# lrjconan/LanczosNetwork

Measured on NVIDIA H100. Metric: QM8 molecules/sec (forward), higher is better.
Workload: dtype f32

## Files before the change

### lanczosnetwork_b200/csrc/sm90.cuh

```cuda
#pragma once
#include <cuda.h>
#include <cuda_runtime.h>
#include <stdint.h>

namespace sm90 {

__device__ __forceinline__ uint32_t smem_u32(const void* p) {
  return static_cast<uint32_t>(__cvta_generic_to_shared(p));
}

__device__ __forceinline__ void mbar_init(uint64_t* bar, uint32_t count) {
  asm volatile("mbarrier.init.shared::cta.b64 [%0], %1;" ::"r"(smem_u32(bar)), "r"(count));
}
__device__ __forceinline__ void fence_barrier_init() {
  asm volatile("fence.mbarrier_init.release.cluster;" ::: "memory");
}
__device__ __forceinline__ void mbar_arrive(uint64_t* bar) {
  asm volatile("mbarrier.arrive.shared::cta.b64 _, [%0];" ::"r"(smem_u32(bar)) : "memory");
}
__device__ __forceinline__ void mbar_arrive_expect_tx(uint64_t* bar, uint32_t bytes) {
  asm volatile("mbarrier.arrive.expect_tx.shared::cta.b64 _, [%0], %1;" ::"r"(smem_u32(bar)),
               "r"(bytes)
               : "memory");
}
// ... 81 lines not shown
        "setp.ne.and.b32 p, %1, 0, e;\n\t"
        "@p mbarrier.arrive.expect_tx.shared::cta.b64 _, [%0], %2;\n\t"
        "@p cp.async.bulk.tensor.2d.shared::cluster.global.mbarrier::complete_tx::bytes"
        " [%3], [%4, {%7, %8}], [%0];\n\t"
        "@p cp.async.bulk.tensor.2d.shared::cluster.global.mbarrier::complete_tx::bytes"
        " [%5], [%6, {%7, %8}], [%0];\n\t}"
        ::"r"(smem_u32(bar)), "r"((uint32_t)pred), "r"(bytes), "r"(smem_u32(dst0)),
          "l"(reinterpret_cast<uint64_t>(m0)), "r"(smem_u32(dst1)), "l"(reinterpret_cast<uint64_t>(m1)),
          "r"(c0), "r"(c1)
        : "memory");
  }
}

__device__ __forceinline__ bool elect_one() {
  uint32_t pred;
  asm volatile(
      "{\n\t.reg .pred p;\n\t"
      "elect.sync _|p, 0xffffffff;\n\t"
      "selp.b32 %0, 1, 0, p;\n\t}"
      : "=r"(pred));
  return pred != 0;
}

__device__ __forceinline__ uint32_t tf32_rna_bits(float v) {
  uint32_t r;
  asm("cvt.rna.tf32.f32 %0, %1;" : "=r"(r) : "f"(v));
  return r;
}

__device__ __forceinline__ uint64_t wgmma_desc_kmajor_sw128(uint32_t smem_addr) {
  uint64_t d = 0;
  d |= (uint64_t)((smem_addr >> 4) & 0x3FFFu);
  d |= (uint64_t)1 << 16;
  d |= (uint64_t)64 << 32;
  d |= (uint64_t)1 << 62;
  return d;
}
__device__ __forceinline__ void wgmma_fence() { asm volatile("wgmma.fence.sync.aligned;" ::: "memory"); }
__device__ __forceinline__ void wgmma_commit() { asm volatile("wgmma.commit_group.sync.aligned;" ::: "memory"); }
__device__ __forceinline__ void wgmma_wait_all() { asm volatile("wgmma.wait_group.sync.aligned 0;" ::: "memory"); }
__device__ __forceinline__ void wgmma_fence_operand(float (&d)[128]) {
#pragma unroll
  for (int i = 0; i < 128; ++i) asm volatile("" : "+f"(d[i])::"memory");
}
__device__ __forceinline__ void wgmma_wait_one() { asm volatile("wgmma.wait_group.sync.aligned 1;" ::: "memory"); }

// ... 47 lines not shown
```

### lanczosnetwork_b200/csrc/spectral_conv_fused.cu

```cuda
#include "tc_gemm.cuh"

namespace {

constexpr int KMAX = 32;
constexpr int GMAX = 32;
constexpr int RMAX = 128;
constexpr int EMAX = 16;
constexpr int FR = 8;

template <bool STAGE>
__global__ void __launch_bounds__(256)
graph_prepare_kernel(const float* __restrict__ L, const float* __restrict__ Q, int N, int E1, int K,
                     float* __restrict__ ell_val, uint8_t* __restrict__ ell_idx,
                     int32_t* __restrict__ ell_max, int32_t* __restrict__ gext, int binarize) {
  extern __shared__ __align__(16) float gp_smem[];
  __shared__ int s_max[EMAX];
  __shared__ int s_ext[2];
  __shared__ uint8_t cnt_s[256 * EMAX];
  const int b = blockIdx.x, tid = threadIdx.x;
  if (tid < EMAX) s_max[tid] = 0;
  if (tid < 2) s_ext[tid] = 0;
  const int64_t per = (int64_t)N * N * E1;
  const float* Lg = L + b * per;
  if (STAGE) {
// ... 375 lines not shown
    if (t < T2) { S[1 + t] = run + ex; tst[t] = run + ex; }
    run += tot;
  }
  if (tid == 0) { S[0] = T2; S[1 + T2] = B; }
  __syncthreads();
  for (int r = warp; r < nrec; r += 32) {
    const int sm = rec_sm[r];
    if (lane < (sm >> 8)) S[T2 + 2 + tst[rec_t[r]] + (sm & 255) + lane] = order[rec_src[r] + lane];
  }
}

constexpr int STACK_PLAIN = 0;
constexpr int STACK_SAGE_MEAN = 1;
constexpr int STACK_SAGE_MAX = 2;
constexpr float SAGE_EPS = 1.1920928955078125e-07f;

template <int kVariant>
struct SpectralPolicyT {
  static constexpr bool kNormRows = kVariant != STACK_PLAIN;
  static constexpr bool kMaxAgg = kVariant == STACK_SAGE_MAX;
  static constexpr bool kLongScales = kVariant == STACK_PLAIN;
  static constexpr int kStagesB = 2;
  static constexpr int kStagesA = 2;
  static constexpr int LMAX = 8;
  struct Params {
    const float* X;
    const int64_t* node_ids;
    const float* emb;
    const float* Q;
    const float* coeff;
    int64_t coeff_stride;
    const float* ell_val;
    const uint8_t* ell_idx;
    const int32_t* ell_max;
    const int32_t* gext;
    const int32_t* tiles;
    const float* bias;
    float* out;
    const float* W_out;
    const float* b_out;
    const float* w_att;
    const float* b_att;
    const uint8_t* mask;
    float* score;
    int P, emb_rows;
    int L;
// ... 31 lines not shown

  struct Tables {
    int ng, Rtot, Ztot, nquads, nzquads, nlines;
    int gid[GMAX];
    int nbase[GMAX + 1], kbase[GMAX + 1], gn[GMAX], gk[GMAX];
    int cnt_e[EMAX], base_e[EMAX], tmax_e[EMAX];
    uint8_t emax[GMAX][EMAX];
    uint8_t row_g[RMAX], row_n[RMAX], z_g[RMAX], z_k[RMAX];
    uint8_t q_g[RMAX / 4 + GMAX], q_n0[RMAX / 4 + GMAX];
    uint8_t zq_g[RMAX / 4 + GMAX], zq_k0[RMAX / 4 + GMAX];
    uint8_t line_e[256], line_t[256];
  };

  const Params& p;
  const int tid, r;
  const int N, K, S, E1, H, XP;
  int Din;
  Tables* tb;
  float* Xs;
  float* Qs;
  float* Ev;
  uint8_t* Ei;
  float fr[FR];
  float u[tcg::BK];
  float* ring;
  tcg::PhaseTimer* ptm = nullptr;

  static __host__ __device__ constexpr size_t tables_bytes() { return (sizeof(Tables) + 15) & ~size_t(15); }

  __device__ SpectralPolicyT(const Params& p_, uint8_t* smem, int tid_)
      : p(p_), tid(tid_), r(tid_ & 127), N(p_.N), K(p_.K), S(p_.S), E1(p_.E1),
        H(p_.H), XP(x_pitch(p_.Din[0], p_.H)), Din(p_.Din[0]) {
    tb = reinterpret_cast<Tables*>(smem);
    Xs = reinterpret_cast<float*>(smem + tables_bytes());
    Qs = Xs + (size_t)RMAX * XP;
    Ev = Qs + (size_t)RMAX * K;
    Ei = reinterpret_cast<uint8_t*>(Ev + (size_t)p.LB * RMAX);
    ring = reinterpret_cast<float*>(tcg::a_ring(smem, kStagesB, kStagesA));
  }
  static size_t smem_fixed(int Din, int K, int H) {
    return (size_t)RMAX * x_pitch(Din, H) * 4 + (size_t)RMAX * K * 4 + tables_bytes() + 16;
  }
  static size_t ell_line_bytes() { return (size_t)RMAX * 5; }
  static size_t readout_bytes(int H, int P, int N) {
    const size_t P1 = (size_t)P + 1, PQ = (P1 + 3) / 4, yr = (RMAX + 1) * P1;
    return (4 * PQ * (H + 4) + yr + ((4 - (yr & 3)) & 3) + H) * 4 + (size_t)GMAX * N;
  }

  __device__ void build_tables(int m_tile) {
    const int lane = tid & 31;
    const int32_t* sc = schedule(p);
// ... 34 lines not shown
        int m = em[e];
        if (lane < ng) tb->emax[lane][e] = (uint8_t)m;
#pragma unroll
        for (int o = 16; o > 0; o >>= 1) m = max(m, __shfl_xor_sync(0xffffffffu, m, o));
        if (lane == 0) tb->tmax_e[e] = m;
      }
    }
    __syncwarp();
    if (lane == 0) {
      tb->ng = ng; tb->Rtot = Rtot; tb->Ztot = Ztot; tb->nquads = nquads; tb->nzquads = nzquads;
      tb->nbase[ng] = Rtot; tb->kbase[ng] = Ztot;
      int left = p.LB, base = 0;
      for (int e = 0; e < E1; ++e) {
        const int c = min(tb->tmax_e[e], left);
        tb->cnt_e[e] = c; tb->base_e[e] = base;
        for (int t = 0; t < c; ++t) { tb->line_e[base + t] = (uint8_t)e; tb->line_t[base + t] = (uint8_t)t; }
        base += c; left -= c;
      }
      tb->nlines = base;
    }
  }

  __device__ void step_begin(int m_tile, int sub, int , tcg::PhaseTimer& tm) {
    tcg::producers_sync();
    const int layer = sub >> 1, step = sub & 1;
    if (step == 1 && S > 0) return;
    Din = p.Din[layer];
    const int warp = tid >> 5, lane = tid & 31;
    constexpr int NW = tcg::PRODUCER_THREADS / 32;
    const int dv = Din / 4;
    ptm = &tm;
    if (layer == 0) {
    if (warp == 0) build_tables(m_tile);
    tcg::producers_sync();
    tm.lap(16);
    const int Rtot = tb->Rtot;
    int64_t my_id = 0;
    if (!p.X && warp + lane * NW < Rtot) {
      const int row = warp + lane * NW;
      my_id = __ldg(p.node_ids + (int64_t)tb->gid[tb->row_g[row]] * N + tb->row_n[row]);
    }
    for (int row = warp, j = 0; row < Rtot; row += NW, ++j) {
      const int64_t src_row = (int64_t)tb->gid[tb->row_g[row]] * N + tb->row_n[row];
      const float* xsrc;
      if (p.X) {
        xsrc = p.X + src_row * Din;
      } else {
        int64_t id = __shfl_sync(0xffffffffu, my_id, j);
        id = id < 0 ? 0 : (id >= p.emb_rows ? p.emb_rows - 1 : id);
        xsrc = p.emb + id * Din;
      }
      float* xd = Xs + (size_t)row * XP;
      for (int q4 = lane; q4 < dv; q4 += 32) sm90::cp_async_16(xd + 4 * q4, xsrc + 4 * q4);
      const float* qsrc = p.Q + src_row * K;
      float* qd = Qs + (size_t)row * K;
      for (int k4 = lane; k4 < (K >> 2); k4 += 32) sm90::cp_async_16(qd + 4 * k4, qsrc + 4 * k4);
    }
// ... 24 lines not shown
          for (int u = 0; u < ELL_BATCH; ++u) {
            const int line = base + u * NW;
            if (line < nlines && rr < Rtot) {
              Ev[(size_t)line * RMAX + rr] = vv[u];
              Ei[(size_t)line * RMAX + rr] = (uint8_t)ii[u];
            }
          }
        }
      }
    }
    tm.lap(18);
    }
    const int Ztot = tb->Ztot;
#pragma unroll
    for (int i = 0; i < FR; ++i) fr[i] = 0.f;
    if (S > 0 && r < Ztot) {
      const float* f = p.coeff + layer * p.coeff_stride + ((int64_t)tb->gid[tb->z_g[r]] * K + tb->z_k[r]) * S;
#pragma unroll
      for (int i = 0; i < FR; ++i)
        if (i < S) fr[i] = __ldg(f + i);
    }
    tm.lap(0);
    sm90::cp_async_wait_all();
    tcg::producers_sync();
    tm.lap(1);
  }

  __device__ __forceinline__ void produce(int sub, int kb, float (&v)[32]) {
#pragma unroll
    for (int j = 0; j < 32; ++j) v[j] = 0.f;
    if (kLongScales && (sub & 1) == 0) {
      if (r >= tb->Ztot) return;
      const int s = kb % S;
      if (s == 0) {
        const int g = tb->z_g[r], n_g = tb->gn[g], nb = tb->nbase[g];
        const float* xs = Xs + (size_t)nb * XP + (kb / S) * tcg::BK;
        const float* qs = Qs + (size_t)nb * K + tb->z_k[r];
#pragma unroll
        for (int j = 0; j < tcg::BK; ++j) u[j] = 0.f;
#pragma unroll 2
        for (int n = 0; n < n_g; ++n) {
          const float q = qs[(size_t)n * K];
          const float4* x4 = reinterpret_cast<const float4*>(xs + (size_t)n * XP);
#pragma unroll
          for (int j = 0; j < 8; ++j) {
            const float4 t = x4[j];
            u[4 * j + 0] = fmaf(q, t.x, u[4 * j + 0]); u[4 * j + 1] = fmaf(q, t.y, u[4 * j + 1]);
            u[4 * j + 2] = fmaf(q, t.z, u[4 * j + 2]); u[4 * j + 3] = fmaf(q, t.w, u[4 * j + 3]);
          }
        }
      }
      float f = 0.f;
      if (S <= FR) {
#pragma unroll
        for (int i = 0; i < FR; ++i) f = (i == s) ? fr[i] : f;
      } else {
        f = __ldg(p.coeff + (sub >> 1) * p.coeff_stride + ((int64_t)tb->gid[tb->z_g[r]] * K + tb->z_k[r]) * S + s);
      }
#pragma unroll
      for (int j = 0; j < tcg::BK; ++j) v[j] = f * u[j];
      return;
    }
    const int j0 = kb * tcg::BK;
    const int c = j0 / Din, d0 = j0 - c * Din;
    if (r >= tb->Rtot) return;
    const int e = c;
    if constexpr (kMaxAgg) {
      produce_max(e, d0, v);
      return;
    }
    const float* xs = Xs + d0;
    const int ts = tb->cnt_e[e], tmax = tb->tmax_e[e];
    const float* ev = Ev + (size_t)tb->base_e[e] * RMAX + r;
    const uint8_t* ei = Ei + (size_t)tb->base_e[e] * RMAX + r;
#pragma unroll 2
    for (int t = 0; t < ts; ++t) {
      const float a = ev[t * RMAX];
      if (a == 0.f) continue;
      const int i = ei[t * RMAX];
      const float4* x4 = reinterpret_cast<const float4*>(xs + (size_t)i * XP);
#pragma unroll
      for (int q = 0; q < 8; ++q) {
        const float4 tt = x4[q];
        v[4 * q + 0] = fmaf(a, tt.x, v[4 * q + 0]);
        v[4 * q + 1] = fmaf(a, tt.y, v[4 * q + 1]);
        v[4 * q + 2] = fmaf(a, tt.z, v[4 * q + 2]);
        v[4 * q + 3] = fmaf(a, tt.w, v[4 * q + 3]);
      }
    }
    if (ts < tmax) {
      const int g = tb->row_g[r], n = tb->row_n[r];
      const int my = tb->emax[g][e], nb = tb->nbase[g];
      const int64_t off0 = (((int64_t)tb->gid[g] * E1 + e) * N) * N + n;
      for (int t = ts; t < tmax; ++t) {
        float a = 0.f;
        int i = 0;
        if (t < my) {
          a = __ldg(p.ell_val + off0 + (int64_t)t * N);
          i = nb + __ldg(p.ell_idx + off0 + (int64_t)t * N);
        }
        if (a == 0.f) continue;
        const float4* x4 = reinterpret_cast<const float4*>(xs + (size_t)i * XP);
#pragma unroll
        for (int q = 0; q < 8; ++q) {
          const float4 tt = x4[q];
          v[4 * q + 0] = fmaf(a, tt.x, v[4 * q + 0]);
          v[4 * q + 1] = fmaf(a, tt.y, v[4 * q + 1]);
          v[4 * q + 2] = fmaf(a, tt.z, v[4 * q + 2]);
          v[4 * q + 3] = fmaf(a, tt.w, v[4 * q + 3]);
        }
      }
    }
  }

  __device__ __forceinline__ void produce_max(int e, int d0, float (&v)[32]) {
#pragma unroll
    for (int j = 0; j < 32; ++j) v[j] = -INFINITY;
    bool any = false;
    const float* xs = Xs + d0;
    const int ts = tb->cnt_e[e], tmax = tb->tmax_e[e];
    const float* ev = Ev + (size_t)tb->base_e[e] * RMAX + r;
    const uint8_t* ei = Ei + (size_t)tb->base_e[e] * RMAX + r;
    for (int t = 0; t < ts; ++t) {
      if (ev[t * RMAX] == 0.f) continue;
      const float4* x4 = reinterpret_cast<const float4*>(xs + (size_t)ei[t * RMAX] * XP);
      any = true;
#pragma unroll
      for (int q = 0; q < 8; ++q) {
        const float4 tt = x4[q];
        v[4 * q + 0] = fmaxf(v[4 * q + 0], tt.x);
        v[4 * q + 1] = fmaxf(v[4 * q + 1], tt.y);
        v[4 * q + 2] = fmaxf(v[4 * q + 2], tt.z);
        v[4 * q + 3] = fmaxf(v[4 * q + 3], tt.w);
      }
    }
    if (ts < tmax) {
      const int g = tb->row_g[r], n = tb->row_n[r];
      const int my = tb->emax[g][e], nb = tb->nbase[g];
      const int64_t off0 = (((int64_t)tb->gid[g] * E1 + e) * N) * N + n;
      for (int t = ts; t < tmax && t < my; ++t) {
        if (__ldg(p.ell_val + off0 + (int64_t)t * N) == 0.f) continue;
        const int i = nb + __ldg(p.ell_idx + off0 + (int64_t)t * N);
        const float4* x4 = reinterpret_cast<const float4*>(xs + (size_t)i * XP);
        any = true;
#pragma unroll
        for (int q = 0; q < 8; ++q) {
          const float4 tt = x4[q];
          v[4 * q + 0] = fmaxf(v[4 * q + 0], tt.x);
          v[4 * q + 1] = fmaxf(v[4 * q + 1], tt.y);
          v[4 * q + 2] = fmaxf(v[4 * q + 2], tt.z);
          v[4 * q + 3] = fmaxf(v[4 * q + 3], tt.w);
        }
      }
    }
    if (!any) {
#pragma unroll
      for (int j = 0; j < 32; ++j) v[j] = 0.f;
    }
  }

  __device__ __forceinline__ void normalize_row(float* row) const {
    float4* r4 = reinterpret_cast<float4*>(row);
    float ss = 0.f;
    for (int h4 = 0; h4 < H / 4; ++h4) {
      const float4 t = r4[h4];
      ss = fmaf(t.x, t.x, ss); ss = fmaf(t.y, t.y, ss); ss = fmaf(t.z, t.z, ss); ss = fmaf(t.w, t.w, ss);
    }
    const float den = sqrtf(ss) + SAGE_EPS;
    for (int h4 = 0; h4 < H / 4; ++h4) {
      const float4 t = r4[h4];
      r4[h4] = make_float4(t.x / den, t.y / den, t.z / den, t.w / den);
    }
  }
  __device__ __forceinline__ float pad_den(const float* bias) const {
    float ss = 0.f;
    for (int h = 0; h < H; ++h) {
      float t = bias ? __ldg(bias + h) : 0.f;
      t = (p.relu != 0) ? fmaxf(t, 0.f) : t;
      ss = fmaf(t, t, ss);
    }
    return sqrtf(ss) + SAGE_EPS;
  }

  __device__ void pre_epilogue(int sub) {
    if ((sub & 1) == 0) return;
    tcg::producers_sync();
    if (ptm) ptm->lap(22);
  }

  static __device__ __forceinline__ bool acc_init(const Params& p, const uint8_t* smem, const float* zr,
                                                  int sub, int row0, int cl, float (&d)[128]) {
    if (!kLongScales || (sub & 1) == 0 || p.S == 0) return false;
    const Tables* tb = reinterpret_cast<const Tables*>(smem);
    const int K = p.K;
    const float* Qs = reinterpret_cast<const float*>(smem + tables_bytes()) + (size_t)RMAX * x_pitch(p.Din[0], p.H);
    const int Rtot = tb->Rtot;
#pragma unroll
    for (int i = 0; i < 128; ++i) d[i] = 0.f;
#pragma unroll
    for (int h = 0; h < 2; ++h) {
      const int row = row0 + 8 * h;
      if (row >= Rtot) continue;
      const int g = tb->row_g[row], k_g = tb->gk[g], zb = tb->kbase[g];
      const float* q = Qs + (size_t)row * K;
      for (int k = 0; k < k_g; ++k) {
        const float a = q[k];
#pragma unroll
        for (int j = 0; j < 16; ++j) {
          const float2 t = *reinterpret_cast<const float2*>(zr + tcg::stg_index(zb + k, 8 * j + cl, tcg::BN));
// ... 8 lines not shown
  __device__ __forceinline__ void store(int sub, int col, float (&x)[tcg::EW]) {
    if (col >= H || r >= tb->Rtot) return;
    float4* o4 = reinterpret_cast<float4*>(Xs + (size_t)r * XP + col);
    const bool relu = p.relu != 0;
    const float* bias = p.bias ? p.bias + (sub >> 1) * H : nullptr;
#pragma unroll
    for (int q = 0; q < tcg::EW / 4; ++q) {
      if (col + 4 * q >= H) break;
      float y[4] = {x[4 * q + 0], x[4 * q + 1], x[4 * q + 2], x[4 * q + 3]};
      if (bias) {
        const float4 b4 = __ldg(reinterpret_cast<const float4*>(bias + col) + q);
        y[0] += b4.x; y[1] += b4.y; y[2] += b4.z; y[3] += b4.w;
      }
      if (relu) { y[0] = fmaxf(y[0], 0.f); y[1] = fmaxf(y[1], 0.f); y[2] = fmaxf(y[2], 0.f); y[3] = fmaxf(y[3], 0.f); }
      o4[q] = make_float4(y[0], y[1], y[2], y[3]);
    }
  }

  __device__ void post_epilogue(int sub) {
    if constexpr (kNormRows) {
      if ((sub & 1) != 0 && r < tb->Rtot) normalize_row(Xs + (size_t)r * XP);
    }
    if ((sub & 1) == 0 || (sub >> 1) != p.L - 1) return;
    tcg::producers_sync();
    if (ptm) ptm->lap(19);
    const int warp = tid >> 5, lane = tid & 31;
    constexpr int NW = tcg::PRODUCER_THREADS / 32;
    const int hv = H / 4, Rtot = tb->Rtot;
    const float* bias = p.bias ? p.bias + (p.L - 1) * H : nullptr;
    if (p.out) {
      for (int row = warp; row < Rtot; row += NW) {
        const float4* src = reinterpret_cast<const float4*>(Xs + (size_t)row * XP);
        float4* dst = reinterpret_cast<float4*>(
            p.out + ((int64_t)tb->gid[tb->row_g[row]] * N + tb->row_n[row]) * H);
        for (int q4 = lane; q4 < hv; q4 += 32) dst[q4] = src[q4];
      }
      if (p.write_pad) {
        [[maybe_unused]] float den = 1.f;
        if constexpr (kNormRows) den = pad_den(bias);
        const int npad = tb->ng * N - Rtot;
        for (int i = warp; i < npad; i += NW) {
          int g = 0, rem = i;
          while (rem >= N - tb->gn[g]) { rem -= N - tb->gn[g]; ++g; }
          float4* dst = reinterpret_cast<float4*>(p.out + ((int64_t)tb->gid[g] * N + tb->gn[g] + rem) * H);
          for (int q4 = lane; q4 < hv; q4 += 32) {
            float y[4];
#pragma unroll
            for (int u = 0; u < 4; ++u) {
              float t = bias ? __ldg(bias + 4 * q4 + u) : 0.f;
              y[u] = (p.relu != 0) ? fmaxf(t, 0.f) : t;
              if constexpr (kNormRows) y[u] = y[u] / den;
            }
            dst[q4] = make_float4(y[0], y[1], y[2], y[3]);
          }
        }
      }
    }
    if (p.score) readout(bias);
  }

  __device__ void readout(const float* bias_last) {
    const int P = p.P, P1 = p.P + 1, PQ = (P1 + 3) >> 2, HP = H + 4;
    float* Wr = ring;
    float* Yr = Wr + (size_t)4 * PQ * HP;
    float* cx = Yr + (size_t)(RMAX + 1) * P1 + ((4 - ((RMAX + 1) * P1 & 3)) & 3);
    for (int e = tid; e < 4 * PQ * H; e += tcg::PRODUCER_THREADS) {
      const int o = e / H, h = e - o * H;
      Wr[o * HP + h] = (o < P) ? __ldg(p.W_out + o * H + h) : (o == P ? __ldg(p.w_att + h) : 0.f);
    }
    [[maybe_unused]] float den = 1.f;
    if constexpr (kNormRows) den = pad_den(bias_last);
    for (int h = tid; h < H; h += tcg::PRODUCER_THREADS) {
      float t = bias_last ? __ldg(bias_last + h) : 0.f;
      cx[h] = (p.relu != 0) ? fmaxf(t, 0.f) : t;
      if constexpr (kNormRows) cx[h] = cx[h] / den;
    }
    uint8_t* mk = reinterpret_cast<uint8_t*>(cx + H);
    for (int e = tid; e < tb->ng * N; e += tcg::PRODUCER_THREADS) {
      const int g = e / N;
      mk[e] = p.mask ? __ldg(p.mask + (int64_t)tb->gid[g] * N + (e - g * N)) : (uint8_t)1;
    }
    tcg::producers_sync();
    if (ptm) ptm->lap(20);
    const int Rtot = tb->Rtot;
    {
      const int warp = tid >> 5, lane = tid & 31;
      const int rb = warp & 3, og = warp >> 2;
      const int per = (P1 + tcg::NGROUPS - 1) / tcg::NGROUPS;
      const int o_end = min(P1, (og + 1) * per);
      const int row = rb * 32 + lane;
      const float4* x4 = reinterpret_cast<const float4*>(Xs + (size_t)(row < Rtot ? row : 0) * XP);
      for (int o0 = og * per; o0 < o_end; o0 += 6) {
        const int cnt = min(6, o_end - o0);
        const float4* w4 = reinterpret_cast<const float4*>(Wr + (size_t)o0 * HP);
        float acc[6] = {0.f, 0.f, 0.f, 0.f, 0.f, 0.f};
#pragma unroll 4
        for (int h4 = 0; h4 < H / 4; ++h4) {
          const float4 x = x4[h4];
#pragma unroll
          for (int j = 0; j < 6; ++j) {
            if (j < cnt) {
              const float4 wv = w4[j * (HP / 4) + h4];
              acc[j] = fmaf(x.x, wv.x, acc[j]); acc[j] = fmaf(x.y, wv.y, acc[j]);
              acc[j] = fmaf(x.z, wv.z, acc[j]); acc[j] = fmaf(x.w, wv.w, acc[j]);
            }
          }
        }
        if (row < Rtot) {
#pragma unroll
          for (int j = 0; j < 6; ++j)
            if (j < cnt) {
              const int o = o0 + j;
              const float v = acc[j] + ((o < P) ? __ldg(p.b_out + o) : __ldg(p.b_att));
              Yr[row * P1 + o] = (o < P) ? v : 1.f / (1.f + expf(-v));
            }
        }
      }
      for (int o = warp; o < P1; o += tcg::PRODUCER_THREADS / 32) {
        float acc = 0.f;
        for (int h = lane; h < H; h += 32) acc = fmaf(cx[h], Wr[o * HP + h], acc);
#pragma unroll
        for (int sh = 16; sh > 0; sh >>= 1) acc += __shfl_xor_sync(0xffffffffu, acc, sh);
        if (lane == 0) {
          const float v = acc + ((o < P) ? __ldg(p.b_out + o) : __ldg(p.b_att));
          Yr[RMAX * P1 + o] = (o < P) ? v : 1.f / (1.f + expf(-v));
        }
      }
    }
    tcg::producers_sync();
    if (ptm) ptm->lap(21);
    for (int e = tid; e < tb->ng * P; e += tcg::PRODUCER_THREADS) {
      const int g = e / P, o = e - g * P;
      const int nb = tb->nbase[g], n_g = tb->gn[g];
      const uint8_t* m = mk + g * N;
      float acc = 0.f;
      int cnt = 0;
      for (int n = 0; n < N; ++n) {
        if (m[n] == 0) continue;
        const float* y = Yr + (n < n_g ? nb + n : RMAX) * P1;
        acc += y[P] * y[o];
        ++cnt;
      }
      p.score[(int64_t)tb->gid[g] * P + o] = acc / (float)cnt;
    }
  }
};
using SpectralPolicy = SpectralPolicyT<STACK_PLAIN>;

}

namespace lnb {
void launch_tile_assign(cudaStream_t s, const int32_t* gext, int B, int K, int32_t* tiles,
                        int32_t* rowmap, int32_t* nrows) {
  const size_t tbytes = ((size_t)6 * (B + 1) + 2 * SCH_NCLS) * sizeof(int32_t);
// ... 132 lines not shown
```

### lanczosnetwork_b200/csrc/tc_gemm.cuh

```cuda
#pragma once
#include "common.cuh"
#include "sm90.cuh"
#include <stdlib.h>
#include <type_traits>

namespace tcg {

constexpr int BM = 128, BN = 128, BK = 32;
constexpr int NGROUPS = 1;
constexpr int TILE_B_BYTES = BN * BK * 4;
constexpr int STAGE_B_BYTES = 2 * TILE_B_BYTES;
constexpr int TILE_A_BYTES = BM * BK * 4;
constexpr int STAGE_A_BYTES = 2 * TILE_A_BYTES;
constexpr int EW = 16;
constexpr int PRODUCER_THREADS = 128 * NGROUPS;
constexpr int CONSUMER_WARP0 = PRODUCER_THREADS / 32;
constexpr int CONSUMER_THREADS = 256;
constexpr int THREADS = PRODUCER_THREADS + CONSUMER_THREADS;
constexpr int MAX_B_STAGES = 6, MAX_A_STAGES = 4;
__host__ __device__ constexpr int core_smem(int stages_b, int stages_a) {
  return stages_b * STAGE_B_BYTES + stages_a * STAGE_A_BYTES + 256;
}
__host__ __device__ constexpr int pass_cols(int stages_a) {
  return stages_a * STAGE_A_BYTES / (BM * 4) < BN ? stages_a * STAGE_A_BYTES / (BM * 4) : BN;
}

__device__ __forceinline__ uint8_t* a_ring(uint8_t* policy_smem, int stages_b, int stages_a) {
  return policy_smem - core_smem(stages_b, stages_a) + stages_b * STAGE_B_BYTES;
}

struct Core {
  uint8_t* Bst;
  uint8_t* Ast;
  uint64_t* b_full;
  uint64_t* b_empty;
  uint64_t* a_full;
  uint64_t* a_empty;
  uint64_t* stg_full;
  uint64_t* stg_empty;
  uint64_t* kept_read;
};

// ... 12 lines not shown
  return c;
}

__device__ unsigned long long* g_prof = nullptr;

struct PhaseTimer {
  unsigned long long* buf;
  long long t0;
  __device__ __forceinline__ void start(int cta, int tid) {
    buf = (tid == 0 && g_prof) ? g_prof + cta * 32 : nullptr;
    if (buf) t0 = clock64();
  }
  __device__ __forceinline__ void start_if(int cta, bool owner) {
    buf = (owner && g_prof) ? g_prof + cta * 32 : nullptr;
    if (buf) t0 = clock64();
  }
  __device__ __forceinline__ void lap(int slot) {
    if (buf) { long long t = clock64(); atomicAdd(&buf[slot], (unsigned long long)(t - t0)); t0 = t; }
  }
};

__device__ __forceinline__ void producers_sync() {
  asm volatile("bar.sync 1, %0;" ::"n"(PRODUCER_THREADS) : "memory");
}
__device__ __forceinline__ void consumers_sync() {
  asm volatile("bar.sync 2, %0;" ::"n"(CONSUMER_THREADS) : "memory");
}

__device__ __forceinline__ int stg_index(int row, int col, int pw) {
  return row * pw + ((((col >> 2) ^ row) & (pw / 4 - 1)) << 2) + (col & 3);
}

template <class P, class = void> struct HasAccInit : std::false_type {};
template <class P> struct HasAccInit<P, std::void_t<decltype(&P::acc_init)>> : std::true_type {};
template <class P, class = void> struct HasOperandFromAcc : std::false_type {};
template <class P> struct HasOperandFromAcc<P, std::void_t<decltype(&P::operand_from_acc)>> : std::true_type {};

template <class Policy>
__device__ __forceinline__ bool next_from_acc(const typename Policy::Params& p, int cta, int ncta, int it,
                                              int nsteps, int& nkb_next) {
  if (it + 1 >= nsteps) return false;
  int m_tile, sub;
  Policy::decode(p, cta, ncta, it + 1, m_tile, sub);
  nkb_next = Policy::num_kblocks(p, sub);
  return Policy::operand_from_acc(p, sub);
}

constexpr int SKIP_MMA = 2;
constexpr int SKIP_TMA = 4;

template <class Policy, int kSkip>
__device__ __forceinline__ void tc_gemm_body(const CUtensorMap& map_hi, const CUtensorMap& map_lo,
                                             const typename Policy::Params& p) {
  extern __shared__ __align__(16) uint8_t smem_raw[];
  const uint32_t pad = (1024u - (sm90::smem_u32(smem_raw) & 1023u)) & 1023u;
  uint8_t* base = smem_raw + pad;
  constexpr int SB = Policy::kStagesB, SA = Policy::kStagesA;
  static_assert(SB >= 1 && SB <= MAX_B_STAGES && SA >= 1 && SA <= MAX_A_STAGES, "ring depths");
  constexpr int PW = pass_cols(SA);
  constexpr int NPASS = BN / PW;
  constexpr bool kAccInit = HasAccInit<Policy>::value;
  static_assert(!kAccInit || NPASS == 1, "a drain kept in the A ring must fit it in one pass");
  constexpr bool kOpAcc = HasOperandFromAcc<Policy>::value;
  constexpr bool kQueue = !kAccInit;
  static_assert(!kOpAcc || SA * BK >= BN, "an operand written from the accumulators needs one A stage per k-block");
  Core c = carve(base, SB, SA);
  uint8_t* policy_smem = base + core_smem(SB, SA);
  float* stg = reinterpret_cast<float*>(c.Ast);

  const int tid = threadIdx.x, warp = tid >> 5, lane = tid & 31;
  const int role = __shfl_sync(0xffffffffu, tid / 128, 0);
  const int cta = blockIdx.x, ncta = gridDim.x;
  const int nsteps = __shfl_sync(0xffffffffu, Policy::num_steps(p, cta, ncta), 0);
  unsigned long long prof_ns0 = 0;
  long long prof_c0 = 0;
  if (tid == 0 && g_prof) {
    asm volatile("mov.u64 %0, %globaltimer;" : "=l"(prof_ns0));
    prof_c0 = clock64();
  }

  if (warp == CONSUMER_WARP0 && lane == 0) {
    sm90::tma_prefetch_desc(&map_hi);
    sm90::tma_prefetch_desc(&map_lo);
    for (int s = 0; s < SB; ++s) {
      sm90::mbar_init(&c.b_full[s], 1);
      sm90::mbar_init(&c.b_empty[s], CONSUMER_THREADS / 32);
    }
    for (int s = 0; s < SA; ++s) {
      sm90::mbar_init(&c.a_full[s], PRODUCER_THREADS);
      sm90::mbar_init(&c.a_empty[s], CONSUMER_THREADS / 32);
    }
    sm90::mbar_init(c.stg_full, CONSUMER_THREADS);
    sm90::mbar_init(c.stg_empty, PRODUCER_THREADS);
    sm90::mbar_init(c.kept_read, CONSUMER_THREADS / 32);
    sm90::fence_barrier_init();
  }
  __syncthreads();

  if (role == 0) {
    const int r = tid & 127;
    Policy pol(p, policy_smem, tid);
    uint32_t cnt = 0;
    uint32_t npass = 0;
    uint32_t nkept = 0;
    bool after_kept = false;
    for (int it = 0; it < nsteps; ++it) {
      int m_tile, sub;
      Policy::decode(p, cta, ncta, it, m_tile, sub);
      int nkb = Policy::num_kblocks(p, sub);
      bool kept = false, to_acc = false;
      if constexpr (kAccInit) kept = Policy::drain_kept(p, sub);
      if constexpr (kOpAcc) {
        if (Policy::operand_from_acc(p, sub)) nkb = 0;
        int nkb_next;
        to_acc = next_from_acc<Policy>(p, cta, ncta, it, nsteps, nkb_next);
      }
      PhaseTimer tm;
      tm.start(cta, tid);
      pol.step_begin(m_tile, sub, 0, tm);
      for (int kb = 0; kb < nkb; ++kb, ++cnt) {
        float v[32];
        if (!(p.dbg & 8)) pol.produce(sub, kb, v);
        const uint32_t sa = cnt % SA;
        if (kAccInit && kb == 0 && after_kept) {
          sm90::mbar_wait(c.kept_read, nkept & 1u);
          ++nkept;
        }
        sm90::mbar_wait(&c.a_empty[sa], ((cnt / SA) & 1u) ^ 1u);
        if (!(p.dbg & 1)) {
          uint8_t* hi = c.Ast + sa * STAGE_A_BYTES + r * 128;
#pragma unroll
          for (int j = 0; j < 8; ++j) {
            uint4 h, l;
            h.x = sm90::tf32_rna_bits(v[4 * j + 0]); h.y = sm90::tf32_rna_bits(v[4 * j + 1]);
            h.z = sm90::tf32_rna_bits(v[4 * j + 2]); h.w = sm90::tf32_rna_bits(v[4 * j + 3]);
            l.x = sm90::tf32_rna_bits(v[4 * j + 0] - __uint_as_float(h.x));
            l.y = sm90::tf32_rna_bits(v[4 * j + 1] - __uint_as_float(h.y));
            l.z = sm90::tf32_rna_bits(v[4 * j + 2] - __uint_as_float(h.z));
            l.w = sm90::tf32_rna_bits(v[4 * j + 3] - __uint_as_float(h.w));
            const int off = (j ^ (r & 7)) * 16;
            *reinterpret_cast<uint4*>(hi + off) = h;
            *reinterpret_cast<uint4*>(hi + TILE_A_BYTES + off) = l;
          }
        }
        sm90::fence_proxy_async();
        sm90::mbar_arrive(&c.a_full[sa]);
      }
      tm.lap((sub & 1) ? 8 : 3);
      pol.pre_epilogue(sub);
      tm.lap(4);
#pragma unroll 1
      for (int q = 0; q < (kept || to_acc ? 0 : NPASS); ++q, ++npass) {
        sm90::mbar_wait(c.stg_full, npass & 1u);
        if (q == 0) tm.lap((sub & 1) ? 9 : 5);
#pragma unroll 1
        for (int col = q * PW; col < (q + 1) * PW; col += EW) {
          float x[EW];
#pragma unroll
          for (int j = 0; j < EW; j += 4) {
            const float4 t = *reinterpret_cast<const float4*>(stg + stg_index(r, col - q * PW + j, PW));
            x[j] = t.x; x[j + 1] = t.y; x[j + 2] = t.z; x[j + 3] = t.w;
          }
          pol.store(sub, col, x);
        }
        sm90::mbar_arrive(c.stg_empty);
      }
      tm.lap(7);
      producers_sync();
      pol.post_epilogue(sub);
      tm.lap(10);
      after_kept = kept;
    }
  } else {
    const int wg = role - 1;
    const int wq = warp & 3;
    float d[128];
    uint32_t cnt = 0, npass = 0;
    uint32_t nacc = 0;
    bool after_kept = false;
    const int row0 = wg * 64 + wq * 16 + (lane >> 2), cl = 2 * (lane & 3);
    const bool w_issuer = warp == CONSUMER_WARP0;
    int l_it = 0, l_kb = 0, l_nkb = -1, l_sub = 0;
    uint32_t l_cnt = 0;
    auto load_next = [&]() {
      while (l_it < nsteps) {
        if (l_nkb < 0) {
          int mt;
          Policy::decode(p, cta, ncta, l_it, mt, l_sub);
          l_nkb = Policy::num_kblocks(p, l_sub);
        }
        if (l_kb < l_nkb) break;
        ++l_it; l_kb = 0; l_nkb = -1;
      }
      if (l_it >= nsteps) return;
      int col0, row0;
      Policy::w_coords(p, l_sub, l_kb, col0, row0);
      const uint32_t st = l_cnt % SB;
      sm90::mbar_wait_uniform(&c.b_empty[st], ((l_cnt / SB) & 1u) ^ 1u);
      uint8_t* dst = c.Bst + st * STAGE_B_BYTES;
      sm90::tma_load_2d_pair_elected<(kSkip & SKIP_TMA) != 0>(w_issuer, &c.b_full[st], STAGE_B_BYTES, dst, &map_hi,
                                                               dst + TILE_B_BYTES, &map_lo, col0, row0);
      ++l_kb; ++l_cnt;
    };
    auto release = [&](uint32_t sb_rel, bool a_stage, uint32_t sa_rel) {
// ... 46 lines not shown
            sm90::wgmma_n128(d, ah, wh, 1u);
            sm90::wgmma_n128_hi(d, ah, sm90::wgmma_desc_kmajor_sw128(b + TILE_B_BYTES + 32 * k), 1u);
            sm90::wgmma_n128_hi(d, sm90::wgmma_desc_kmajor_sw128(a_lo + 32 * k), wh, 1u);
          }
          sm90::wgmma_commit();
          if constexpr (kQueue) sm90::wgmma_wait_one();
          else sm90::wgmma_wait_all();
          sm90::wgmma_fence_operand(d);
        }
        if constexpr (kQueue) {
          if (kb > 0) release((cnt - 1) % SB, !from_acc, from_acc ? (uint32_t)(kb - 1) : (acnt - 1) % SA);
        } else {
          release(sb, !from_acc, sa);
        }
      }
      if constexpr (!(kSkip & SKIP_MMA)) {
        sm90::wgmma_wait_all();
        sm90::wgmma_fence_operand(d);
      }
      if (kQueue && nkb > 0)
        release((cnt - 1) % SB, !from_acc, from_acc ? (uint32_t)(nkb - 1) : (cnt - nacc - 1) % SA);
      if (from_acc) nacc += nkb;
      PhaseTimer ctm;
      if (to_acc) ctm.start_if(cta, tid == PRODUCER_THREADS);
      consumers_sync();
      if (to_acc) {
        if constexpr (kOpAcc) {
#pragma unroll
          for (int i = 0; i < 64; i += 2) {
            const int col = 8 * (i / 4) + cl, row = row0 + 8 * ((i / 2) % 2), kb = i / 16;
            if (kb < nkb_next) {
              const float y0 = Policy::acc_operand(p, policy_smem, sub, col, d[i] + d[i + 64]);
              const float y1 = Policy::acc_operand(p, policy_smem, sub, col + 1, d[i + 1] + d[i + 65]);
              uint2 h, l;
              h.x = sm90::tf32_rna_bits(y0); h.y = sm90::tf32_rna_bits(y1);
              l.x = sm90::tf32_rna_bits(y0 - __uint_as_float(h.x));
              l.y = sm90::tf32_rna_bits(y1 - __uint_as_float(h.y));
              uint8_t* dst = c.Ast + kb * STAGE_A_BYTES + row * 128 + (((((col & 31) >> 2) ^ row) & 7) << 4) +
                             (col & 3) * 4;
              *reinterpret_cast<uint2*>(dst) = h;
              *reinterpret_cast<uint2*>(dst + TILE_A_BYTES) = l;
            }
          }
          sm90::fence_proxy_async();
          consumers_sync();
          ctm.lap(14);
        }
// ... 7 lines not shown
            if (col >= q * PW && col < (q + 1) * PW)
              *reinterpret_cast<float2*>(stg + stg_index(row, col - q * PW, PW)) =
                  make_float2(d[i] + d[i + 64], d[i + 1] + d[i + 65]);
          }
          if (!kept) sm90::mbar_arrive(c.stg_full);
        }
      }
      if (kept) consumers_sync();
      after_kept = kept;
    }
  }

  __syncthreads();
  if (tid == 0 && g_prof) {
    unsigned long long ns1;
    asm volatile("mov.u64 %0, %globaltimer;" : "=l"(ns1));
    atomicAdd(&g_prof[cta * 32 + 11], ns1 - prof_ns0);
    atomicAdd(&g_prof[cta * 32 + 12], (unsigned long long)(clock64() - prof_c0));
    g_prof[cta * 32 + 13] = prof_ns0;
  }
}

template <class Policy>
__global__ void __launch_bounds__(THREADS, 1)
tc_gemm_kernel(const __grid_constant__ CUtensorMap map_hi,
               const __grid_constant__ CUtensorMap map_lo, const typename Policy::Params p) {
  tc_gemm_body<Policy, 0>(map_hi, map_lo, p);
}

template <class Policy, int kSkip>
__global__ void __launch_bounds__(THREADS, 1)
tc_gemm_probe_kernel(const __grid_constant__ CUtensorMap map_hi,
                     const __grid_constant__ CUtensorMap map_lo, const typename Policy::Params p) {
  tc_gemm_body<Policy, kSkip>(map_hi, map_lo, p);
}

__device__ __forceinline__ void store_row_chunk(float* orow, int ncols, const float* bias, bool relu,
                                                int col, const float (&x)[EW]) {
  if (orow == nullptr || col >= ncols) return;
  const bool vec_ok = (reinterpret_cast<uintptr_t>(orow + col) & 15) == 0;
#pragma unroll
  for (int j = 0; j < EW; j += 4) {
    float o[4];
#pragma unroll
    for (int u = 0; u < 4; ++u) {
      const int n = col + j + u;
      float y = x[j + u];
      if (n < ncols) {
        if (bias) y += __ldg(bias + n);
        if (relu) y = fmaxf(y, 0.f);
      }
      o[u] = y;
    }
    if (vec_ok && col + j + 3 < ncols) {
// ... 61 lines not shown
  cudaError_t e = cudaMemcpyToSymbol(g_prof, &buf, sizeof(buf));
  if (e != cudaSuccess) { lnb::set_err("%s: %s", who, cudaGetErrorString(e)); return (int)e; }
  g_prof_mirrored = buf;
  return LNB_OK;
}

template <class Pol>
static int launch(lnb_stream_t stream, const float* W_hi, const float* W_lo, int w_rows, int w_cols,
                  size_t smem, int items, const typename Pol::Params& p, const char* who) {
  CUtensorMap map_hi, map_lo;
  int rc = make_weight_map(&map_hi, W_hi, w_rows, w_cols, who);
  if (rc != LNB_OK) return rc;
  rc = make_weight_map(&map_lo, W_lo, w_rows, w_cols, who);
  if (rc != LNB_OK) return rc;
  rc = sync_prof_buffer(who);
  if (rc != LNB_OK) return rc;
  const int skip = p.dbg & (SKIP_MMA | SKIP_TMA);
  auto kern = skip == 0                    ? tc_gemm_kernel<Pol>
              : skip == SKIP_MMA           ? tc_gemm_probe_kernel<Pol, SKIP_MMA>
              : skip == SKIP_TMA           ? tc_gemm_probe_kernel<Pol, SKIP_TMA>
                                           : tc_gemm_probe_kernel<Pol, SKIP_MMA | SKIP_TMA>;
  cudaFuncSetAttribute(kern, cudaFuncAttributeMaxDynamicSharedMemorySize, (int)smem);
  const int grid = items < sm_count() ? items : sm_count();
  kern<<<grid, THREADS, smem, (cudaStream_t)stream>>>(map_hi, map_lo, p);
  lnb::count_launch();
  return lnb::finish_launch(who);
}

}
```

Baseline: 1.072 million.

## Split spectral producer work across two warpgroups with register rebalancing

For the plain spectral variant, the A-operand producer role grows to two warpgroups, and each one computes half of the k-block columns. The staging epilogue loop is split between them, and setmaxnreg moves registers from producers to consumers. The goal is to double the throughput of the CUDA-core aggregation that feeds the wgmma consumers. This adds 128 threads per CTA and lowers the producer register budget, which could spill. It also changes NW and the readout loop partitioning, and any policy that assumed a single group could break.

```diff
diff --git a/lanczosnetwork_b200/csrc/sm90.cuh b/lanczosnetwork_b200/csrc/sm90.cuh
--- a/lanczosnetwork_b200/csrc/sm90.cuh
+++ b/lanczosnetwork_b200/csrc/sm90.cuh
@@ -127,6 +127,15 @@
   return pred != 0;
 }
 
+template <int kRegs>
+__device__ __forceinline__ void setmaxnreg_dec() {
+  asm volatile("setmaxnreg.dec.sync.aligned.u32 %0;" ::"n"(kRegs));
+}
+template <int kRegs>
+__device__ __forceinline__ void setmaxnreg_inc() {
+  asm volatile("setmaxnreg.inc.sync.aligned.u32 %0;" ::"n"(kRegs));
+}
+
 __device__ __forceinline__ uint32_t tf32_rna_bits(float v) {
   uint32_t r;
   asm("cvt.rna.tf32.f32 %0, %1;" : "=r"(r) : "f"(v));
diff --git a/lanczosnetwork_b200/csrc/spectral_conv_fused.cu b/lanczosnetwork_b200/csrc/spectral_conv_fused.cu
--- a/lanczosnetwork_b200/csrc/spectral_conv_fused.cu
+++ b/lanczosnetwork_b200/csrc/spectral_conv_fused.cu
@@ -421,6 +421,10 @@
   static constexpr bool kLongScales = kVariant == STACK_PLAIN;
   static constexpr int kStagesB = 2;
   static constexpr int kStagesA = 2;
+  static constexpr int kProducerGroups = kNormRows ? 1 : 2;
+  static constexpr int kPT = 128 * kProducerGroups;
+  static constexpr int kCols = tcg::BK / kProducerGroups;
+  static_assert(!kNormRows || kProducerGroups == 1, "normalize_row() runs on rows its thread stored whole");
   static constexpr int LMAX = 8;
   struct Params {
     const float* X;
@@ -498,11 +502,12 @@
   float* Ev;
   uint8_t* Ei;
   float fr[FR];
-  float u[tcg::BK];
+  float u[kCols];
   float* ring;
   tcg::PhaseTimer* ptm = nullptr;
 
   static __host__ __device__ constexpr size_t tables_bytes() { return (sizeof(Tables) + 15) & ~size_t(15); }
+  __device__ __forceinline__ int part_col() const { return kProducerGroups == 1 ? 0 : (tid >> 7) * kCols; }
 
   __device__ SpectralPolicyT(const Params& p_, uint8_t* smem, int tid_)
       : p(p_), tid(tid_), r(tid_ & 127), N(p_.N), K(p_.K), S(p_.S), E1(p_.E1),
@@ -583,17 +588,17 @@
   }
 
   __device__ void step_begin(int m_tile, int sub, int , tcg::PhaseTimer& tm) {
-    tcg::producers_sync();
+    tcg::producers_sync<kPT>();
     const int layer = sub >> 1, step = sub & 1;
     if (step == 1 && S > 0) return;
     Din = p.Din[layer];
     const int warp = tid >> 5, lane = tid & 31;
-    constexpr int NW = tcg::PRODUCER_THREADS / 32;
+    constexpr int NW = kPT / 32;
     const int dv = Din / 4;
     ptm = &tm;
     if (layer == 0) {
     if (warp == 0) build_tables(m_tile);
-    tcg::producers_sync();
+    tcg::producers_sync<kPT>();
     tm.lap(16);
     const int Rtot = tb->Rtot;
     int64_t my_id = 0;
@@ -664,28 +669,28 @@
     }
     tm.lap(0);
     sm90::cp_async_wait_all();
-    tcg::producers_sync();
+    tcg::producers_sync<kPT>();
     tm.lap(1);
   }
 
-  __device__ __forceinline__ void produce(int sub, int kb, float (&v)[32]) {
-#pragma unroll
-    for (int j = 0; j < 32; ++j) v[j] = 0.f;
+  __device__ __forceinline__ void produce(int sub, int kb, float (&v)[kCols]) {
+#pragma unroll
+    for (int j = 0; j < kCols; ++j) v[j] = 0.f;
     if (kLongScales && (sub & 1) == 0) {
       if (r >= tb->Ztot) return;
       const int s = kb % S;
       if (s == 0) {
         const int g = tb->z_g[r], n_g = tb->gn[g], nb = tb->nbase[g];
-        const float* xs = Xs + (size_t)nb * XP + (kb / S) * tcg::BK;
+        const float* xs = Xs + (size_t)nb * XP + (kb / S) * tcg::BK + part_col();
         const float* qs = Qs + (size_t)nb * K + tb->z_k[r];
 #pragma unroll
-        for (int j = 0; j < tcg::BK; ++j) u[j] = 0.f;
+        for (int j = 0; j < kCols; ++j) u[j] = 0.f;
 #pragma unroll 2
         for (int n = 0; n < n_g; ++n) {
           const float q = qs[(size_t)n * K];
           const float4* x4 = reinterpret_cast<const float4*>(xs + (size_t)n * XP);
 #pragma unroll
-          for (int j = 0; j < 8; ++j) {
+          for (int j = 0; j < kCols / 4; ++j) {
             const float4 t = x4[j];
             u[4 * j + 0] = fmaf(q, t.x, u[4 * j + 0]); u[4 * j + 1] = fmaf(q, t.y, u[4 * j + 1]);
             u[4 * j + 2] = fmaf(q, t.z, u[4 * j + 2]); u[4 * j + 3] = fmaf(q, t.w, u[4 * j + 3]);
@@ -700,7 +705,7 @@
         f = __ldg(p.coeff + (sub >> 1) * p.coeff_stride + ((int64_t)tb->gid[tb->z_g[r]] * K + tb->z_k[r]) * S + s);
       }
 #pragma unroll
-      for (int j = 0; j < tcg::BK; ++j) v[j] = f * u[j];
+      for (int j = 0; j < kCols; ++j) v[j] = f * u[j];
       return;
     }
     const int j0 = kb * tcg::BK;
@@ -711,7 +716,7 @@
       produce_max(e, d0, v);
       return;
     }
-    const float* xs = Xs + d0;
+    const float* xs = Xs + d0 + part_col();
     const int ts = tb->cnt_e[e], tmax = tb->tmax_e[e];
     const float* ev = Ev + (size_t)tb->base_e[e] * RMAX + r;
     const uint8_t* ei = Ei + (size_t)tb->base_e[e] * RMAX + r;
@@ -722,7 +727,7 @@
       const int i = ei[t * RMAX];
       const float4* x4 = reinterpret_cast<const float4*>(xs + (size_t)i * XP);
 #pragma unroll
-      for (int q = 0; q < 8; ++q) {
+      for (int q = 0; q < kCols / 4; ++q) {
         const float4 tt = x4[q];
         v[4 * q + 0] = fmaf(a, tt.x, v[4 * q + 0]);
         v[4 * q + 1] = fmaf(a, tt.y, v[4 * q + 1]);
@@ -744,7 +749,7 @@
         if (a == 0.f) continue;
         const float4* x4 = reinterpret_cast<const float4*>(xs + (size_t)i * XP);
 #pragma unroll
-        for (int q = 0; q < 8; ++q) {
+        for (int q = 0; q < kCols / 4; ++q) {
           const float4 tt = x4[q];
           v[4 * q + 0] = fmaf(a, tt.x, v[4 * q + 0]);
           v[4 * q + 1] = fmaf(a, tt.y, v[4 * q + 1]);
@@ -755,11 +760,11 @@
     }
   }
 
-  __device__ __forceinline__ void produce_max(int e, int d0, float (&v)[32]) {
-#pragma unroll
-    for (int j = 0; j < 32; ++j) v[j] = -INFINITY;
+  __device__ __forceinline__ void produce_max(int e, int d0, float (&v)[kCols]) {
+#pragma unroll
+    for (int j = 0; j < kCols; ++j) v[j] = -INFINITY;
     bool any = false;
-    const float* xs = Xs + d0;
+    const float* xs = Xs + d0 + part_col();
     const int ts = tb->cnt_e[e], tmax = tb->tmax_e[e];
     const float* ev = Ev + (size_t)tb->base_e[e] * RMAX + r;
     const uint8_t* ei = Ei + (size_t)tb->base_e[e] * RMAX + r;
@@ -768,7 +773,7 @@
       const float4* x4 = reinterpret_cast<const float4*>(xs + (size_t)ei[t * RMAX] * XP);
       any = true;
 #pragma unroll
-      for (int q = 0; q < 8; ++q) {
+      for (int q = 0; q < kCols / 4; ++q) {
         const float4 tt = x4[q];
         v[4 * q + 0] = fmaxf(v[4 * q + 0], tt.x);
         v[4 * q + 1] = fmaxf(v[4 * q + 1], tt.y);
@@ -786,7 +791,7 @@
         const float4* x4 = reinterpret_cast<const float4*>(xs + (size_t)i * XP);
         any = true;
 #pragma unroll
-        for (int q = 0; q < 8; ++q) {
+        for (int q = 0; q < kCols / 4; ++q) {
           const float4 tt = x4[q];
           v[4 * q + 0] = fmaxf(v[4 * q + 0], tt.x);
           v[4 * q + 1] = fmaxf(v[4 * q + 1], tt.y);
@@ -797,7 +802,7 @@
     }
     if (!any) {
 #pragma unroll
-      for (int j = 0; j < 32; ++j) v[j] = 0.f;
+      for (int j = 0; j < kCols; ++j) v[j] = 0.f;
     }
   }
 
@@ -826,7 +831,7 @@
 
   __device__ void pre_epilogue(int sub) {
     if ((sub & 1) == 0) return;
-    tcg::producers_sync();
+    tcg::producers_sync<kPT>();
     if (ptm) ptm->lap(22);
   }
 
@@ -881,10 +886,10 @@
       if ((sub & 1) != 0 && r < tb->Rtot) normalize_row(Xs + (size_t)r * XP);
     }
     if ((sub & 1) == 0 || (sub >> 1) != p.L - 1) return;
-    tcg::producers_sync();
+    tcg::producers_sync<kPT>();
     if (ptm) ptm->lap(19);
     const int warp = tid >> 5, lane = tid & 31;
-    constexpr int NW = tcg::PRODUCER_THREADS / 32;
+    constexpr int NW = kPT / 32;
     const int hv = H / 4, Rtot = tb->Rtot;
     const float* bias = p.bias ? p.bias + (p.L - 1) * H : nullptr;
     if (p.out) {
@@ -923,29 +928,29 @@
     float* Wr = ring;
     float* Yr = Wr + (size_t)4 * PQ * HP;
     float* cx = Yr + (size_t)(RMAX + 1) * P1 + ((4 - ((RMAX + 1) * P1 & 3)) & 3);
-    for (int e = tid; e < 4 * PQ * H; e += tcg::PRODUCER_THREADS) {
+    for (int e = tid; e < 4 * PQ * H; e += kPT) {
       const int o = e / H, h = e - o * H;
       Wr[o * HP + h] = (o < P) ? __ldg(p.W_out + o * H + h) : (o == P ? __ldg(p.w_att + h) : 0.f);
     }
     [[maybe_unused]] float den = 1.f;
     if constexpr (kNormRows) den = pad_den(bias_last);
-    for (int h = tid; h < H; h += tcg::PRODUCER_THREADS) {
+    for (int h = tid; h < H; h += kPT) {
       float t = bias_last ? __ldg(bias_last + h) : 0.f;
       cx[h] = (p.relu != 0) ? fmaxf(t, 0.f) : t;
       if constexpr (kNormRows) cx[h] = cx[h] / den;
     }
     uint8_t* mk = reinterpret_cast<uint8_t*>(cx + H);
-    for (int e = tid; e < tb->ng * N; e += tcg::PRODUCER_THREADS) {
+    for (int e = tid; e < tb->ng * N; e += kPT) {
       const int g = e / N;
       mk[e] = p.mask ? __ldg(p.mask + (int64_t)tb->gid[g] * N + (e - g * N)) : (uint8_t)1;
     }
-    tcg::producers_sync();
+    tcg::producers_sync<kPT>();
     if (ptm) ptm->lap(20);
     const int Rtot = tb->Rtot;
     {
       const int warp = tid >> 5, lane = tid & 31;
       const int rb = warp & 3, og = warp >> 2;
-      const int per = (P1 + tcg::NGROUPS - 1) / tcg::NGROUPS;
+      const int per = (P1 + kProducerGroups - 1) / kProducerGroups;
       const int o_end = min(P1, (og + 1) * per);
       const int row = rb * 32 + lane;
       const float4* x4 = reinterpret_cast<const float4*>(Xs + (size_t)(row < Rtot ? row : 0) * XP);
@@ -975,7 +980,7 @@
             }
         }
       }
-      for (int o = warp; o < P1; o += tcg::PRODUCER_THREADS / 32) {
+      for (int o = warp; o < P1; o += kPT / 32) {
         float acc = 0.f;
         for (int h = lane; h < H; h += 32) acc = fmaf(cx[h], Wr[o * HP + h], acc);
 #pragma unroll
@@ -986,9 +991,9 @@
         }
       }
     }
-    tcg::producers_sync();
+    tcg::producers_sync<kPT>();
     if (ptm) ptm->lap(21);
-    for (int e = tid; e < tb->ng * P; e += tcg::PRODUCER_THREADS) {
+    for (int e = tid; e < tb->ng * P; e += kPT) {
       const int g = e / P, o = e - g * P;
       const int nb = tb->nbase[g], n_g = tb->gn[g];
       const uint8_t* m = mk + g * N;
diff --git a/lanczosnetwork_b200/csrc/tc_gemm.cuh b/lanczosnetwork_b200/csrc/tc_gemm.cuh
--- a/lanczosnetwork_b200/csrc/tc_gemm.cuh
+++ b/lanczosnetwork_b200/csrc/tc_gemm.cuh
@@ -18,6 +18,21 @@
 constexpr int CONSUMER_THREADS = 256;
 constexpr int THREADS = PRODUCER_THREADS + CONSUMER_THREADS;
 constexpr int MAX_B_STAGES = 6, MAX_A_STAGES = 4;
+constexpr int PRODUCER_REGS_2G = 88, CONSUMER_REGS_2G = 168;
+static_assert(256 * PRODUCER_REGS_2G + CONSUMER_THREADS * CONSUMER_REGS_2G == 65536, "register file");
+
+template <class P, class = void> struct ProducerGroups : std::integral_constant<int, NGROUPS> {};
+template <class P>
+struct ProducerGroups<P, std::void_t<decltype(P::kProducerGroups)>> : std::integral_constant<int, P::kProducerGroups> {};
+template <class P> struct CtaRoles {
+  static constexpr int G = ProducerGroups<P>::value;
+  static_assert(G == 1 || G == 2, "one or two producer warpgroups");
+  static constexpr int PT = 128 * G;
+  static constexpr int CW0 = PT / 32;
+  static constexpr int THREADS = PT + CONSUMER_THREADS;
+  static constexpr int AV = BK / G;
+  static __device__ __forceinline__ int part(int tid) { return G == 1 ? 0 : tid >> 7; }
+};
 __host__ __device__ constexpr int core_smem(int stages_b, int stages_a) {
   return stages_b * STAGE_B_BYTES + stages_a * STAGE_A_BYTES + 256;
 }
@@ -76,6 +91,10 @@
 
 __device__ __forceinline__ void producers_sync() {
   asm volatile("bar.sync 1, %0;" ::"n"(PRODUCER_THREADS) : "memory");
+}
+template <int kProducerThreads>
+__device__ __forceinline__ void producers_sync() {
+  asm volatile("bar.sync 1, %0;" ::"n"(kProducerThreads) : "memory");
 }
 __device__ __forceinline__ void consumers_sync() {
   asm volatile("bar.sync 2, %0;" ::"n"(CONSUMER_THREADS) : "memory");
@@ -118,6 +137,7 @@
   constexpr bool kOpAcc = HasOperandFromAcc<Policy>::value;
   constexpr bool kQueue = !kAccInit;
   static_assert(!kOpAcc || SA * BK >= BN, "an operand written from the accumulators needs one A stage per k-block");
+  using Roles = CtaRoles<Policy>;
   Core c = carve(base, SB, SA);
   uint8_t* policy_smem = base + core_smem(SB, SA);
   float* stg = reinterpret_cast<float*>(c.Ast);
@@ -133,7 +153,7 @@
     prof_c0 = clock64();
   }
 
-  if (warp == CONSUMER_WARP0 && lane == 0) {
+  if (warp == Roles::CW0 && lane == 0) {
     sm90::tma_prefetch_desc(&map_hi);
     sm90::tma_prefetch_desc(&map_lo);
     for (int s = 0; s < SB; ++s) {
@@ -141,17 +161,18 @@
       sm90::mbar_init(&c.b_empty[s], CONSUMER_THREADS / 32);
     }
     for (int s = 0; s < SA; ++s) {
-      sm90::mbar_init(&c.a_full[s], PRODUCER_THREADS);
+      sm90::mbar_init(&c.a_full[s], Roles::PT);
       sm90::mbar_init(&c.a_empty[s], CONSUMER_THREADS / 32);
     }
     sm90::mbar_init(c.stg_full, CONSUMER_THREADS);
-    sm90::mbar_init(c.stg_empty, PRODUCER_THREADS);
+    sm90::mbar_init(c.stg_empty, Roles::PT);
     sm90::mbar_init(c.kept_read, CONSUMER_THREADS / 32);
     sm90::fence_barrier_init();
   }
   __syncthreads();
 
-  if (role == 0) {
+  if (Roles::G == 1 ? role == 0 : role < Roles::G) {
+    if constexpr (Roles::G == 2) sm90::setmaxnreg_dec<PRODUCER_REGS_2G>();
     const int r = tid & 127;
     Policy pol(p, policy_smem, tid);
     uint32_t cnt = 0;
@@ -173,7 +194,7 @@
       tm.start(cta, tid);
       pol.step_begin(m_tile, sub, 0, tm);
       for (int kb = 0; kb < nkb; ++kb, ++cnt) {
-        float v[32];
+        float v[Roles::AV];
         if (!(p.dbg & 8)) pol.produce(sub, kb, v);
         const uint32_t sa = cnt % SA;
         if (kAccInit && kb == 0 && after_kept) {
@@ -184,16 +205,16 @@
         if (!(p.dbg & 1)) {
           uint8_t* hi = c.Ast + sa * STAGE_A_BYTES + r * 128;
 #pragma unroll
-          for (int j = 0; j < 8; ++j) {
-            uint4 h, l;
-            h.x = sm90::tf32_rna_bits(v[4 * j + 0]); h.y = sm90::tf32_rna_bits(v[4 * j + 1]);
-            h.z = sm90::tf32_rna_bits(v[4 * j + 2]); h.w = sm90::tf32_rna_bits(v[4 * j + 3]);
-            l.x = sm90::tf32_rna_bits(v[4 * j + 0] - __uint_as_float(h.x));
-            l.y = sm90::tf32_rna_bits(v[4 * j + 1] - __uint_as_float(h.y));
-            l.z = sm90::tf32_rna_bits(v[4 * j + 2] - __uint_as_float(h.z));
-            l.w = sm90::tf32_rna_bits(v[4 * j + 3] - __uint_as_float(h.w));
-            const int off = (j ^ (r & 7)) * 16;
-            *reinterpret_cast<uint4*>(hi + off) = h;
+          for (int j = 0; j < Roles::AV / 4; ++j) {
+            uint4 hv, l;
+            hv.x = sm90::tf32_rna_bits(v[4 * j + 0]); hv.y = sm90::tf32_rna_bits(v[4 * j + 1]);
+            hv.z = sm90::tf32_rna_bits(v[4 * j + 2]); hv.w = sm90::tf32_rna_bits(v[4 * j + 3]);
+            l.x = sm90::tf32_rna_bits(v[4 * j + 0] - __uint_as_float(hv.x));
+            l.y = sm90::tf32_rna_bits(v[4 * j + 1] - __uint_as_float(hv.y));
+            l.z = sm90::tf32_rna_bits(v[4 * j + 2] - __uint_as_float(hv.z));
+            l.w = sm90::tf32_rna_bits(v[4 * j + 3] - __uint_as_float(hv.w));
+            const int off = ((Roles::part(tid) * (Roles::AV / 4) + j) ^ (r & 7)) * 16;
+            *reinterpret_cast<uint4*>(hi + off) = hv;
             *reinterpret_cast<uint4*>(hi + TILE_A_BYTES + off) = l;
           }
         }
@@ -208,7 +229,7 @@
         sm90::mbar_wait(c.stg_full, npass & 1u);
         if (q == 0) tm.lap((sub & 1) ? 9 : 5);
 #pragma unroll 1
-        for (int col = q * PW; col < (q + 1) * PW; col += EW) {
+        for (int col = q * PW + Roles::part(tid) * EW; col < (q + 1) * PW; col += Roles::G * EW) {
           float x[EW];
 #pragma unroll
           for (int j = 0; j < EW; j += 4) {
@@ -220,20 +241,21 @@
         sm90::mbar_arrive(c.stg_empty);
       }
       tm.lap(7);
-      producers_sync();
+      producers_sync<Roles::PT>();
       pol.post_epilogue(sub);
       tm.lap(10);
       after_kept = kept;
     }
   } else {
-    const int wg = role - 1;
+    if constexpr (Roles::G == 2) sm90::setmaxnreg_inc<CONSUMER_REGS_2G>();
+    const int wg = role - Roles::G;
     const int wq = warp & 3;
     float d[128];
     uint32_t cnt = 0, npass = 0;
     uint32_t nacc = 0;
     bool after_kept = false;
     const int row0 = wg * 64 + wq * 16 + (lane >> 2), cl = 2 * (lane & 3);
-    const bool w_issuer = warp == CONSUMER_WARP0;
+    const bool w_issuer = warp == Roles::CW0;
     int l_it = 0, l_kb = 0, l_nkb = -1, l_sub = 0;
     uint32_t l_cnt = 0;
     auto load_next = [&]() {
@@ -326,7 +348,7 @@
         release((cnt - 1) % SB, !from_acc, from_acc ? (uint32_t)(nkb - 1) : (cnt - nacc - 1) % SA);
       if (from_acc) nacc += nkb;
       PhaseTimer ctm;
-      if (to_acc) ctm.start_if(cta, tid == PRODUCER_THREADS);
+      if (to_acc) ctm.start_if(cta, tid == Roles::PT);
       consumers_sync();
       if (to_acc) {
         if constexpr (kOpAcc) {
@@ -380,14 +402,14 @@
 }
 
 template <class Policy>
-__global__ void __launch_bounds__(THREADS, 1)
+__global__ void __launch_bounds__(CtaRoles<Policy>::THREADS, 1)
 tc_gemm_kernel(const __grid_constant__ CUtensorMap map_hi,
                const __grid_constant__ CUtensorMap map_lo, const typename Policy::Params p) {
   tc_gemm_body<Policy, 0>(map_hi, map_lo, p);
 }
 
 template <class Policy, int kSkip>
-__global__ void __launch_bounds__(THREADS, 1)
+__global__ void __launch_bounds__(CtaRoles<Policy>::THREADS, 1)
 tc_gemm_probe_kernel(const __grid_constant__ CUtensorMap map_hi,
                      const __grid_constant__ CUtensorMap map_lo, const typename Policy::Params p) {
   tc_gemm_body<Policy, kSkip>(map_hi, map_lo, p);
@@ -495,7 +517,7 @@
                                            : tc_gemm_probe_kernel<Pol, SKIP_MMA | SKIP_TMA>;
   cudaFuncSetAttribute(kern, cudaFuncAttributeMaxDynamicSharedMemorySize, (int)smem);
   const int grid = items < sm_count() ? items : sm_count();
-  kern<<<grid, THREADS, smem, (cudaStream_t)stream>>>(map_hi, map_lo, p);
+  kern<<<grid, CtaRoles<Pol>::THREADS, smem, (cudaStream_t)stream>>>(map_hi, map_lo, p);
   lnb::count_launch();
   return lnb::finish_launch(who);
 }
```

Result: no change. 1.087 million (median of 6 runs) (+1.4%).
